# sanderslab/magellanmapper

Measured on AMD Instinct MI355X. Metric: Mvoxels/s, 2048x2048x1024 uint16 stack, 5-sigma LoG blob detection, higher is better.
Workload: dtype f16x2 MFMA (f32 accumulate) + 16-bit fixed-point intermediates; f64 re-score of every candidate

## Files before the change

magellanmapper_amd/csrc/mmx_fused4.hip:

```cpp

#include <algorithm>
#include <type_traits>

#include "mmx_common.h"

typedef _Float16 h2_4 __attribute__((ext_vector_type(2)));
typedef _Float16 h8_4 __attribute__((ext_vector_type(8)));
typedef float f2_4 __attribute__((ext_vector_type(2)));
typedef float f4_4 __attribute__((ext_vector_type(4)));
typedef unsigned u4_4 __attribute__((ext_vector_type(4)));
typedef unsigned u2_4 __attribute__((ext_vector_type(2)));

#define MMX_ZX4_MAXCLS 8
#ifndef ZX4_ST_AUX
#define ZX4_ST_AUX 0
#endif
#ifndef ZX4_LD_AUX
#define ZX4_LD_AUX 0
#endif

struct mmx_zx4_cfg {
    float w0[MMX_MAX_RADIUS_FAST + 1];
    float w2[MMX_MAX_RADIUS_FAST + 1];
    float xscale;
    int radius;
    int ncw, ncz;
    int wcls[MMX_ZX4_MAXCLS];
    int zcls[MMX_ZX4_MAXCLS];
    int maxcol, maxu;
    float qp, qq;
    int staged;
    int ntw;
};

namespace {

#ifndef ZX4_PF
#define ZX4_PF 3
#endif
constexpr int kPF4 = ZX4_PF;
#ifndef ZX6_PF
#define ZX6_PF 2
#endif
constexpr float kLoScale = 2048.f;
constexpr float kLoInv = 1.f / 2048.f;

using rsrc4_t = __amdgpu_buffer_rsrc_t;
__device__ __forceinline__ rsrc4_t make_rsrc4(const void* p)
{
    return __builtin_amdgcn_make_buffer_rsrc(const_cast<void*>(p), 0, 0x7fffffff, 0x00020000);
}

template <int NKX, int LA> struct cls4 {
    static constexpr int R8 = NKX == 1 ? 8 : (LA == 1 ? 16 : 24);
    static __host__ __device__ constexpr int xstart(int c)
    {
        const int lo = 16 * c - R8;
        const int al = lo & ~31;
        return (al + 32 * NKX >= 16 * c + 16 + R8) ? al : lo;
    }
    static constexpr int NKZ = LA + 1;
    static constexpr int NT = 2 * NKZ;
};

__device__ __forceinline__ unsigned pack_h2(float a, float b)
{
    const f2_4 v = {a, b};
    return __builtin_bit_cast(unsigned, __builtin_convertvector(v, h2_4));
}

__device__ __forceinline__ float folded_tap(const float* w, int R, int p, int o, int n)
{
    float s = 0.f;
    int d = p - o; d = d < 0 ? -d : d;
    if (d <= R) s += w[d];
    d = (-1 - p) - o; d = d < 0 ? -d : d;
    if (d <= R) s += w[d];
    d = (2 * n - 1 - p) - o; d = d < 0 ? -d : d;
    if (d <= R) s += w[d];
    return s;
}

template <int NKX, int LA>
__global__ void __launch_bounds__(256)
zx4_setup(mmx_zx4_cfg cfg, u4_4* __restrict__ xtab, u4_4* __restrict__ ztab)
{
    using cg = cls4<NKX, LA>;
    const int R = cfg.radius;
    const int lane = threadIdx.x & 63;
    const int kq = lane >> 4, col = lane & 15;
    const int e = blockIdx.x * 4 + (threadIdx.x >> 6);
    const int nx_entries = cfg.ncw * cfg.maxcol * NKX * 2;
    const int nz_entries = cfg.ncz * cfg.maxu * cg::NKZ * 2;
    float wt[8];
    u4_4* dst;
    if (e < nx_entries) {
        const int kern = e & 1;
        const int m = (e >> 1) % NKX;
        const int c = ((e >> 1) / NKX) % cfg.maxcol;
        const int cl = ((e >> 1) / NKX) / cfg.maxcol;
        const int W = cfg.wcls[cl];
        const float* w = kern ? cfg.w2 : cfg.w0;
        const int xo = 16 * c + col;
        const int cwin = cfg.ntw == 2 ? (c & ~1) : c;
        const int xc = (cfg.staged == 2 ? 16 * cwin - cg::R8 : cg::xstart(c)) + 32 * m + 8 * kq;
        int xl = xc < 0 ? 0 : xc;
        xl = xl > W - 8 ? W - 8 : xl;
        if (cfg.staged) xl = xc;
#pragma unroll
        for (int j = 0; j < 8; ++j) {
            const int p = xl + j;
            const bool ok = p >= xc && p < xc + 8 && p >= 0 && p < W && xo < W;
            wt[j] = ok ? folded_tap(w, R, p, xo, W) * cfg.xscale * (cfg.qp > 0.f ? (kern ? cfg.qq : cfg.qp) : 1.f) : 0.f;
        }
        dst = xtab + (size_t)e * 2 * 64;
    } else if (e < nx_entries + nz_entries) {
        const int ez = e - nx_entries;
        const int kern = ez & 1;
        const int ks = (ez >> 1) % cg::NKZ;
        const int U = ((ez >> 1) / cg::NKZ) % cfg.maxu;
        const int cl = ((ez >> 1) / cg::NKZ) / cfg.maxu;
        const int nz = cfg.zcls[cl];
        const float* w = kern ? cfg.w2 : cfg.w0;
        const int zo = 16 * U + col;
#pragma unroll
        for (int j = 0; j < 8; ++j) {
            const int i = 2 * ks + (j >> 2);
            const int zi = 16 * (U - LA + i) + 4 * kq + (j & 3);
            const bool ok = i < cg::NT - 1 && zi >= 0 && zi < nz && zo < nz;
            wt[j] = ok ? folded_tap(w, R, zi, zo, nz) * (cfg.qp > 0.f && kern ? cfg.qq / cfg.qp : 1.f) : 0.f;
        }
        dst = ztab + (size_t)ez * 2 * 64;
    } else {
        return;
    }
    unsigned hi[4], lo[4];
#pragma unroll
    for (int j = 0; j < 8; j += 2) {
        const f2_4 v = {wt[j], wt[j + 1]};
        const h2_4 h = __builtin_convertvector(v, h2_4);
        const f2_4 r = {(wt[j] - (float)h.x) * kLoScale, (wt[j + 1] - (float)h.y) * kLoScale};
        hi[j >> 1] = __builtin_bit_cast(unsigned, h);
        lo[j >> 1] = __builtin_bit_cast(unsigned, __builtin_convertvector(r, h2_4));
    }
    dst[lane] = (u4_4){hi[0], hi[1], hi[2], hi[3]};
    dst[64 + lane] = (u4_4){lo[0], lo[1], lo[2], lo[3]};
}

template <typename InT> struct pieces4;
template <> struct pieces4<uint16_t> {
    using raw_t = u4_4;
    static __device__ __forceinline__ raw_t load(rsrc4_t r, unsigned off, unsigned soff = 0)
    {
        return __builtin_bit_cast(u4_4, __builtin_amdgcn_raw_buffer_load_b128(r, off, soff, ZX4_LD_AUX));
    }
    static __device__ __forceinline__ void split(const raw_t& d, u4_4& hi, u4_4& lo)
    {
        const h2_4 four = {(_Float16)4.0f, (_Float16)4.0f};
        const h2_4 sixty4th = {(_Float16)0.015625f, (_Float16)0.015625f};
#pragma unroll
        for (int i = 0; i < 4; ++i) {
            const unsigned th = __builtin_amdgcn_perm(0x44004400u, d[i], 0x07030501u);
            const unsigned tl = __builtin_amdgcn_perm(0x24002400u, d[i], 0x07020500u);
            hi[i] = __builtin_bit_cast(unsigned, __builtin_bit_cast(h2_4, th) - four);
            lo[i] = __builtin_bit_cast(unsigned, __builtin_bit_cast(h2_4, tl) - sixty4th);
        }
    }
    static constexpr float kBiasHi = 4.0f, kBiasLo = 0.015625f;
    static __device__ __forceinline__ void split_biased(const raw_t& d, u4_4& hi, u4_4& lo)
    {
#pragma unroll
        for (int i = 0; i < 4; ++i) {
            hi[i] = __builtin_amdgcn_perm(0x44004400u, d[i], 0x07030501u);
            lo[i] = __builtin_amdgcn_perm(0x24002400u, d[i], 0x07020500u);
        }
    }
};

struct presplit_t { u4_4 h, l; };
template <> struct pieces4<float> {
    using raw_t = presplit_t;
    static __device__ __forceinline__ raw_t load(rsrc4_t r, unsigned off, unsigned soff = 0)
    {
        raw_t v;
        v.h = __builtin_bit_cast(u4_4, __builtin_amdgcn_raw_buffer_load_b128(r, off, soff, ZX4_LD_AUX));
        v.l = __builtin_bit_cast(u4_4, __builtin_amdgcn_raw_buffer_load_b128(r, off + 256u, soff, ZX4_LD_AUX));
        return v;
    }
    static __device__ __forceinline__ void split(const raw_t& d, u4_4& hi, u4_4& lo) { hi = d.h; lo = d.l; }
    [[maybe_unused]] static constexpr float kBiasHi = 0.f, kBiasLo = 0.f;
    static __device__ __forceinline__ void split_biased(const raw_t& d, u4_4& hi, u4_4& lo) { hi = d.h; lo = d.l; }
};
template <typename InT> struct is_f32_4 { static constexpr bool value = false; };
template <> struct is_f32_4<float> { static constexpr bool value = true; };
template <typename InT> struct lo_scaled4 { static constexpr bool value = false; };
template <> struct lo_scaled4<float> { static constexpr bool value = true; };

__device__ __forceinline__ f4_4 mfma16(const u4_4& a, const u4_4& b, const f4_4& c)
{
    return __builtin_amdgcn_mfma_f32_16x16x32_f16(__builtin_bit_cast(h8_4, a), __builtin_bit_cast(h8_4, b), c, 0, 0, 0);
}

template <int NKX, int LA, typename InT, bool Q16 = false, int NTW = 1>
__global__ void __launch_bounds__(256, (NTW == 1 && (LA == 1 || Q16) && !is_f32_4<InT>::value) ? 3 : 2)
zx4_kernel(const InT* __restrict__ vol, int64_t stride_z, int64_t stride_y,
           const mmx_block* __restrict__ blocks, int64_t slot_elems,
           float* __restrict__ gp, float* __restrict__ gq,
           const u4_4* __restrict__ xtab, const u4_4* __restrict__ ztab, mmx_zx4_cfg cfg)
{
    using cg = cls4<NKX, LA>;
    using pc = pieces4<InT>;
    constexpr int NKZ = cg::NKZ, NT = cg::NT;
    constexpr int kUnit = std::is_same<InT, float>::value ? 512 : 256;
    constexpr bool LO_SCALED = lo_scaled4<InT>::value;
    static_assert(NTW == 1 || (NTW == 2 && Q16 && NKX == 2 && LA == 1), "two tiles per wave: 16-bit tiles, 8 < radius <= 16");
    constexpr bool ZLDS = LA == 1 || Q16;
    constexpr int PF = ZLDS ? ZX6_PF : kPF4;
    const mmx_block bd = blocks[blockIdx.y];
    const int W = bd.nx, nz = bd.nz;
    const int ntx = (W + 15) >> 4;
    const int bx = (int)(blockIdx.x & 7) * (int)(gridDim.x >> 3) + (int)(blockIdx.x >> 3);
    const int gw = bx * 4 + __builtin_amdgcn_readfirstlane((int)(threadIdx.x >> 6));
    const int ntp = (ntx + NTW - 1) / NTW;
    const int y = gw / ntp;
    const int c = (gw - y * ntp) * NTW;
    const int lane = threadIdx.x & 63;
    const int li = lane & 15, kq = lane >> 4;
    int cw = 0, cz = 0;
    for (int i = 1; i < cfg.ncw; ++i) cw = cfg.wcls[i] == W ? i : cw;
    for (int i = 1; i < cfg.ncz; ++i) cz = cfg.zcls[i] == nz ? i : cz;
    const int ntz = (nz + 15) >> 4;
    const int R = cfg.radius;
    const int u_lo = (R + 15) >> 4;
    const int u_hi = (nz - 16 - R) >> 4;
    const u4_4* zt = ztab + ((size_t)cz * cfg.maxu * NKZ * 2) * 128 + lane;
    constexpr bool ROT = ZLDS && Q16 && NTW == 1 && !is_f32_4<InT>::value && (NKX == 1 || LA == 2);
    constexpr int ZL1 = NKZ * 4 * 64;
    __shared__ u4_4 zl[ZLDS ? (ROT ? 2 : 1) * ZL1 : 1];
    if constexpr (ZLDS) {
        const u4_4* zi = ztab + ((size_t)(cz * cfg.maxu + (u_lo < cfg.maxu ? u_lo : 0)) * NKZ * 2) * 128;
        for (int e = threadIdx.x; e < ZL1; e += 256) zl[e] = zi[e];
        __syncthreads();
        if constexpr (ROT) {
            for (int e = threadIdx.x; e < ZL1; e += 256) {
                const u4_4 cur = zl[e];
                const u4_4 prev = e >= 256 ? zl[e - 256] : (u4_4){0u, 0u, 0u, 0u};
                zl[ZL1 + e] = (u4_4){prev.z, prev.w, cur.x, cur.y};
            }
            __syncthreads();
        }
    }
    if (y >= bd.ny) return;

    u4_4 xw[NTW][NKX][2][2];
    const bool has2 = NTW == 2 && c + 1 < ntx;
#pragma unroll
    for (int i = 0; i < NTW; ++i) {
        const u4_4* xt = xtab + ((size_t)(cw * cfg.maxcol + (i && !has2 ? c : c + i)) * NKX * 2) * 128 + lane;
#pragma unroll
        for (int m = 0; m < NKX; ++m)
#pragma unroll
            for (int k = 0; k < 2; ++k) {
                xw[i][m][k][0] = xt[(m * 2 + k) * 128];
                xw[i][m][k][1] = xt[(m * 2 + k) * 128 + 64];
            }
    }
    constexpr bool BIASED = Q16 && !is_f32_4<InT>::value && LA == 1;
    constexpr bool MIXSPLIT = Q16;
    const f4_4 zero4 = {0.f, 0.f, 0.f, 0.f};
    f4_4 a_start[NTW], b_start[NTW];
#pragma unroll
    for (int i = 0; i < NTW; ++i) { a_start[i] = zero4; b_start[i] = zero4; }
    if constexpr (BIASED) {
        const u4_4 ones = {0x3C003C00u, 0x3C003C00u, 0x3C003C00u, 0x3C003C00u};
#pragma unroll
        for (int i = 0; i < NTW; ++i) {
            f4_4 sh[2] = {zero4, zero4}, sl[2] = {zero4, zero4};
#pragma unroll
            for (int m = 0; m < NKX; ++m)
#pragma unroll
                for (int k = 0; k < 2; ++k) {
                    sh[k] = mfma16(ones, xw[i][m][k][0], sh[k]);
                    sl[k] = mfma16(ones, xw[i][m][k][1], sl[k]);
                }
            const float ca = -((pc::kBiasHi + pc::kBiasLo) * sh[0][0] + pc::kBiasHi * sl[0][0] * kLoInv);
            const float cb = -((pc::kBiasHi + pc::kBiasLo) * sh[1][0] + pc::kBiasHi * sl[1][0] * kLoInv);
            a_start[i] = (f4_4){ca, ca, ca, ca};
            b_start[i] = (f4_4){cb, cb, cb, cb};
        }
    }
    u4_4 zw[ZLDS ? 1 : NKZ][2][2];
    int zset = -1;

    const InT* in = vol + (int64_t)bd.slot * stride_z;
    const int nch8 = (W + 7) >> 3;
    unsigned xoff[NKX];
#pragma unroll
    for (int m = 0; m < NKX; ++m) {
        int j = 2 * c - cg::R8 / 8 + 4 * m + kq;
        j = j < 0 ? 0 : (j > nch8 - 1 ? nch8 - 1 : j);
        xoff[m] = (unsigned)(j * kUnit + li * 16);
    }
    const rsrc4_t rin = make_rsrc4(in);
    auto load_tile = [&](int t, typename pc::raw_t (&raw)[NKX]) __attribute__((always_inline)) {
        const unsigned so = (unsigned)((y * ntz + t) * nch8) * (unsigned)kUnit;
#pragma unroll
        for (int m = 0; m < NKX; ++m) raw[m] = pc::load(rin, xoff[m], so);
    };

    unsigned win[NTW][4][NT][2];
#pragma unroll
    for (int w = 0; w < NTW; ++w)
#pragma unroll
        for (int a = 0; a < 4; ++a)
#pragma unroll
            for (int i = 0; i < NT; ++i) { win[w][a][i][0] = 0u; win[w][a][i][1] = 0u; }

    const unsigned col_b = (unsigned)ntz * 1024u;
    const unsigned live_b = col_b - (unsigned)(16 * ntz - nz) * 64u;
    const int64_t wave_e = (int64_t)((y * ntx + c) * ntz) * 256;
    const rsrc4_t rp = __builtin_amdgcn_make_buffer_rsrc(gp + (int64_t)bd.slot * slot_elems + wave_e, 0, (int)live_b, 0x00020000);
    const rsrc4_t rq = __builtin_amdgcn_make_buffer_rsrc(gq + (int64_t)bd.slot * slot_elems + wave_e, 0, (int)live_b, 0x00020000);
    const rsrc4_t rp2 = __builtin_amdgcn_make_buffer_rsrc(gp + (int64_t)bd.slot * slot_elems + wave_e + (int64_t)ntz * 256, 0,
                                                          has2 ? (int)live_b : 0, 0x00020000);
    const unsigned plane_b = 64u;
    unsigned obase = (unsigned)((4 * li + kq) * 16);

    typename pc::raw_t raw[PF][NKX];
#pragma unroll
    for (int u = 0; u < PF; ++u) load_tile(u < ntz ? u : ntz - 1, raw[u]);

    f4_4 outP[PF][NTW], outQ[PF];
#pragma unroll
    for (int u = 0; u < PF; ++u) {
#pragma unroll
        for (int w = 0; w < NTW; ++w) outP[u][w] = zero4;
        outQ[u] = zero4;
    }
    auto step = [&](int t, auto steady_tag, auto phase_tag, typename pc::raw_t (&rw)[NKX], f4_4 (&P)[NTW], f4_4& Q) __attribute__((always_inline)) {
        constexpr bool STEADY = decltype(steady_tag)::value;
        constexpr int PH = decltype(phase_tag)::value;
        constexpr bool TURN = STEADY && ROT && PH >= 0;
        constexpr int SLOT = TURN ? PH : 2 * LA;
        if constexpr (!TURN) {
#pragma unroll
            for (int w = 0; w < NTW; ++w)
#pragma unroll
                for (int a = 0; a < 4; ++a)
#pragma unroll
                    for (int i = 0; i < 2 * LA; ++i) { win[w][a][i][0] = win[w][a][i + 1][0]; win[w][a][i][1] = win[w][a][i + 1][1]; }
        }
        if (STEADY || t < ntz) {
            u4_4 dh[NKX], dl[NKX];
#pragma unroll
            for (int m = 0; m < NKX; ++m) {
                if constexpr (BIASED) pc::split_biased(rw[m], dh[m], dl[m]);
                else pc::split(rw[m], dh[m], dl[m]);
            }
            __builtin_amdgcn_sched_barrier(0);
            if (STEADY) load_tile(t + PF < ntz ? t + PF : ntz - 1, rw);
            else if (t + PF < ntz) load_tile(t + PF, rw);
            __builtin_amdgcn_sched_barrier(0);
#pragma unroll
            for (int w = 0; w < NTW; ++w) {
                f4_4 a0 = a_start[w], a1 = zero4, b0 = b_start[w], b1 = zero4;
#pragma unroll
                for (int m = 0; m < NKX; ++m) {
                    a0 = mfma16(dh[m], xw[w][m][0][0], a0);
                    b0 = mfma16(dh[m], xw[w][m][1][0], b0);
                    a1 = mfma16(dh[m], xw[w][m][0][1], a1);
                    b1 = mfma16(dh[m], xw[w][m][1][1], b1);
                    if constexpr (LO_SCALED) {
                        a1 = mfma16(dl[m], xw[w][m][0][0], a1);
                        b1 = mfma16(dl[m], xw[w][m][1][0], b1);
                    } else {
                        a0 = mfma16(dl[m], xw[w][m][0][0], a0);
                        b0 = mfma16(dl[m], xw[w][m][1][0], b0);
                        if constexpr (!Q16) {
                            a1 = mfma16(dl[m], xw[w][m][0][1], a1);
                            b1 = mfma16(dl[m], xw[w][m][1][1], b1);
                        }
                    }
                }
#pragma unroll
                for (int r = 0; r < 4; r += 2) {
                    const float av0 = __builtin_fmaf(a1[r], kLoInv, a0[r]), av1 = __builtin_fmaf(a1[r + 1], kLoInv, a0[r + 1]);
                    const float bv0 = __builtin_fmaf(b1[r], kLoInv, b0[r]), bv1 = __builtin_fmaf(b1[r + 1], kLoInv, b0[r + 1]);
                    const f2_4 av = {av0, av1}, bv = {bv0, bv1};
                    const h2_4 ah = __builtin_convertvector(av, h2_4), bh = __builtin_convertvector(bv, h2_4);
                    if constexpr (MIXSPLIT) {
                        const f2_4 ar = {av0 - (float)ah.x, av1 - (float)ah.y}, br = {bv0 - (float)bh.x, bv1 - (float)bh.y};
                        win[w][0][SLOT][r >> 1] = __builtin_bit_cast(unsigned, ah);
                        win[w][1][SLOT][r >> 1] = __builtin_bit_cast(unsigned, __builtin_convertvector(ar, h2_4));
                        win[w][2][SLOT][r >> 1] = __builtin_bit_cast(unsigned, bh);
                        win[w][3][SLOT][r >> 1] = __builtin_bit_cast(unsigned, __builtin_convertvector(br, h2_4));
                        continue;
                    }
                    const f2_4 ar = {__builtin_fmaf((float)ah.x, -kLoScale, av0 * kLoScale), __builtin_fmaf((float)ah.y, -kLoScale, av1 * kLoScale)};
                    const f2_4 br = {__builtin_fmaf((float)bh.x, -kLoScale, bv0 * kLoScale), __builtin_fmaf((float)bh.y, -kLoScale, bv1 * kLoScale)};
                    win[w][0][SLOT][r >> 1] = __builtin_bit_cast(unsigned, ah);
                    win[w][1][SLOT][r >> 1] = __builtin_bit_cast(unsigned, __builtin_convertvector(ar, h2_4));
                    win[w][2][SLOT][r >> 1] = __builtin_bit_cast(unsigned, bh);
                    win[w][3][SLOT][r >> 1] = __builtin_bit_cast(unsigned, __builtin_convertvector(br, h2_4));
                }
            }
        } else {
#pragma unroll
            for (int w = 0; w < NTW; ++w)
#pragma unroll
                for (int a = 0; a < 4; ++a) { win[w][a][SLOT][0] = 0u; win[w][a][SLOT][1] = 0u; }
        }
        const int U = t - LA;
        if (STEADY || U >= 0) {
            const int want = (U >= u_lo && U <= u_hi) ? u_lo : U;
            if constexpr (!STEADY && !ZLDS) {
                if (want != zset) {
                    zset = want;
#pragma unroll
                    for (int ks = 0; ks < NKZ; ++ks)
#pragma unroll
                        for (int k = 0; k < 2; ++k) {
                            zw[ks][k][0] = zt[((size_t)(want * NKZ + ks) * 2 + k) * 128];
                            zw[ks][k][1] = zt[((size_t)(want * NKZ + ks) * 2 + k) * 128 + 64];
                        }
                }
            }
            f4_4 p0[NTW], p1[NTW], q0[NTW], q1[NTW];
#pragma unroll
            for (int w = 0; w < NTW; ++w) { p0[w] = zero4; p1[w] = zero4; q0[w] = zero4; q1[w] = zero4; }
#pragma unroll
            for (int ks = 0; ks < NKZ; ++ks) {
                u4_4 z00, z01, z10, z11;
                if constexpr (!ZLDS) {
                    z00 = zw[ks][0][0]; z01 = zw[ks][0][1]; z10 = zw[ks][1][0]; z11 = zw[ks][1][1];
                } else if constexpr (STEADY) {
                    constexpr int TR = TURN ? (PH - (NT - 2) + NT) % NT : 0;
                    const int KF = ((TR & 1) ? ZL1 : 0) + ((ks - TR / 2 + NKZ) % NKZ) * 256;
                    z00 = zl[KF + 0 * 64 + lane]; z01 = zl[KF + 1 * 64 + lane];
                    z10 = zl[KF + 2 * 64 + lane]; z11 = zl[KF + 3 * 64 + lane];
                } else {
                    const u4_4* zp = zt + ((size_t)(want * NKZ + ks) * 2) * 128;
                    z00 = zp[0]; z01 = zp[64]; z10 = zp[128]; z11 = zp[192];
                }
#pragma unroll
                for (int w = 0; w < NTW; ++w) {
                    const u4_4 ah = {win[w][0][2 * ks][0], win[w][0][2 * ks][1], win[w][0][2 * ks + 1][0], win[w][0][2 * ks + 1][1]};
                    const u4_4 al = {win[w][1][2 * ks][0], win[w][1][2 * ks][1], win[w][1][2 * ks + 1][0], win[w][1][2 * ks + 1][1]};
                    const u4_4 bh = {win[w][2][2 * ks][0], win[w][2][2 * ks][1], win[w][2][2 * ks + 1][0], win[w][2][2 * ks + 1][1]};
                    const u4_4 bl = {win[w][3][2 * ks][0], win[w][3][2 * ks][1], win[w][3][2 * ks + 1][0], win[w][3][2 * ks + 1][1]};
                    p0[w] = mfma16(ah, z00, p0[w]);
                    q0[w] = mfma16(bh, z00, q0[w]);
                    p1[w] = mfma16(ah, z01, p1[w]);
                    q1[w] = mfma16(bh, z01, q1[w]);
                    if constexpr (MIXSPLIT) {
                        p0[w] = mfma16(al, z00, p0[w]);
                        q0[w] = mfma16(bl, z00, q0[w]);
                    } else {
                        p1[w] = mfma16(al, z00, p1[w]);
                        q1[w] = mfma16(bl, z00, q1[w]);
                    }
                    q0[w] = mfma16(ah, z10, q0[w]);
                    q1[w] = mfma16(ah, z11, q1[w]);
                    if constexpr (MIXSPLIT) q0[w] = mfma16(al, z10, q0[w]);
                    else q1[w] = mfma16(al, z10, q1[w]);
                }
                if constexpr (ZLDS && !STEADY) __builtin_amdgcn_sched_barrier(0);
            }
            __builtin_amdgcn_sched_barrier(0);
#pragma unroll
            for (int w = 0; w < NTW; ++w) asm volatile("" ::"v"(P[w]));
            asm volatile("" ::"v"(Q));
            {
                if constexpr (Q16) {
#pragma unroll
                    for (int w = 0; w < NTW; ++w) {
#pragma unroll
                        for (int r = 0; r < 4; r += 2) {
                            const float pa = __builtin_fmaf(p1[w][r], kLoInv, p0[w][r]), pb = __builtin_fmaf(p1[w][r + 1], kLoInv, p0[w][r + 1]);
                            const float qa = __builtin_fmaf(q1[w][r], kLoInv, q0[w][r]), qb = __builtin_fmaf(q1[w][r + 1], kLoInv, q0[w][r + 1]);
                            const unsigned pu = __builtin_bit_cast(unsigned, __builtin_amdgcn_cvt_pknorm_u16(pa, pb));
                            const unsigned qs = __builtin_bit_cast(unsigned, __builtin_amdgcn_cvt_pknorm_i16(qa, qb));
                            const unsigned da = __builtin_amdgcn_perm(qs, pu, 0x05040100u);
                            const unsigned db = __builtin_amdgcn_perm(qs, pu, 0x07060302u);
                            float ra, rb;
                            asm volatile("v_mov_b32 %0, %1" : "=v"(ra) : "v"(__uint_as_float(da)));
                            asm volatile("v_mov_b32 %0, %1" : "=v"(rb) : "v"(__uint_as_float(db)));
                            P[w][r] = ra;
                            P[w][r + 1] = rb;
                        }
                        if (w == 0) __builtin_amdgcn_raw_buffer_store_b128(__builtin_bit_cast(u4_4, P[w]), rp, obase, 0, ZX4_ST_AUX);
                        else __builtin_amdgcn_raw_buffer_store_b128(__builtin_bit_cast(u4_4, P[w]), rp2, obase, 0, ZX4_ST_AUX);
                    }
                } else {
#pragma unroll
                for (int r = 0; r < 4; ++r) {
                    const float pv = __builtin_fmaf(p1[0][r], kLoInv, p0[0][r]);
                    const float qv = __builtin_fmaf(q1[0][r], kLoInv, q0[0][r]);
                    float pr, qr;
                    asm volatile("v_mov_b32 %0, %1" : "=v"(pr) : "v"(pv));
                    asm volatile("v_mov_b32 %0, %1" : "=v"(qr) : "v"(qv));
                    P[0][r] = pr;
                    Q[r] = qr;
                }
                __builtin_amdgcn_raw_buffer_store_b128(__builtin_bit_cast(u4_4, P[0]), rp, obase, 0, ZX4_ST_AUX);
                __builtin_amdgcn_raw_buffer_store_b128(__builtin_bit_cast(u4_4, Q), rq, obase, 0, ZX4_ST_AUX);
                }
            }
            obase += 16u * plane_b;
        }
        __builtin_amdgcn_sched_barrier(0);
    };
    const int t_end = ntz + LA;
    int tA = ((u_lo + LA + PF - 1) / PF) * PF;
    int nB = (u_hi + LA + 1 < ntz ? u_hi + LA + 1 : ntz) - tA;
    constexpr int GROUP = ROT ? NT : PF;
    static_assert(GROUP % PF == 0, "a turn of the window is a whole number of rings");
    nB = nB > 0 ? (nB / GROUP) * GROUP : 0;
    if (tA > t_end) tA = ((t_end + PF - 1) / PF) * PF;
    const int tB = tA + nB;
#pragma unroll 1
    for (int t0 = 0; t0 < tA; t0 += PF) {
#pragma unroll
        for (int u = 0; u < PF; ++u)
            if (t0 + u < t_end) step(t0 + u, std::false_type{}, std::integral_constant<int, -1>{}, raw[u], outP[u], outQ[u]);
    }
    if (nB > 0) {
        if (!ZLDS && zset != u_lo) {
            zset = u_lo;
#pragma unroll
            for (int ks = 0; ks < NKZ; ++ks)
#pragma unroll
                for (int k = 0; k < 2; ++k) {
                    zw[ks][k][0] = zt[((size_t)(u_lo * NKZ + ks) * 2 + k) * 128];
                    zw[ks][k][1] = zt[((size_t)(u_lo * NKZ + ks) * 2 + k) * 128 + 64];
                }
        }
        __builtin_amdgcn_s_waitcnt(0x0F70);
        auto turn = [&](int t0, auto... J) __attribute__((always_inline)) {
            (step(t0 + decltype(J)::value, std::true_type{},
                  std::integral_constant<int, ROT ? (NT - 1 + decltype(J)::value) % NT : -1>{},
                  raw[decltype(J)::value % PF], outP[decltype(J)::value % PF], outQ[decltype(J)::value % PF]), ...);
        };
        if constexpr (!ROT) {
#pragma unroll 1
            for (int t0 = tA; t0 < tB; t0 += PF) {
#pragma unroll
                for (int u = 0; u < PF; ++u) step(t0 + u, std::true_type{}, std::integral_constant<int, -1>{}, raw[u], outP[u], outQ[u]);
            }
        } else {
#pragma unroll 1
            for (int t0 = tA; t0 < tB; t0 += GROUP) {
                using std::integral_constant;
                if constexpr (GROUP == 4) turn(t0, integral_constant<int, 0>{}, integral_constant<int, 1>{}, integral_constant<int, 2>{},
                                               integral_constant<int, 3>{});
                else turn(t0, integral_constant<int, 0>{}, integral_constant<int, 1>{}, integral_constant<int, 2>{},
                          integral_constant<int, 3>{}, integral_constant<int, 4>{}, integral_constant<int, 5>{});
                static_assert(GROUP == 4 || GROUP == 6, "turn lengths built: 4 (radius <= 16), 6 (radius <= 24)");
            }
        }
    }
#pragma unroll 1
    for (int t0 = tB; t0 < t_end; t0 += PF) {
#pragma unroll
        for (int u = 0; u < PF; ++u)
            if (t0 + u < t_end) step(t0 + u, std::false_type{}, std::integral_constant<int, -1>{}, raw[u], outP[u], outQ[u]);
    }
}



template <typename InT>
__global__ void __launch_bounds__(256)
zx6_pack_kernel(const InT* __restrict__ vol, int64_t stride_z, int64_t stride_y, int64_t stride_x,
                const mmx_block* __restrict__ blocks, uint16_t* __restrict__ pack, int64_t pack_stride)
{
    constexpr int PITCH = 512 + 8;
    __shared__ __attribute__((aligned(16))) uint16_t tile[16][PITCH];
    const mmx_block bd = blocks[blockIdx.y];
    const int ntz = (bd.nz + 15) >> 4, nch8 = (bd.nx + 7) >> 3;
    const int yt = blockIdx.x;
    if (yt >= bd.ny * ntz) return;
    const int y = yt / ntz, t = yt - y * ntz;
    const int wave = threadIdx.x >> 6, lane = threadIdx.x & 63;
    const InT* src = vol + bd.src_off + (int64_t)y * stride_y;
    bool quads = false;
    if constexpr (sizeof(InT) == 2)
        quads = stride_x == 1 && ((bd.src_off | stride_y | stride_z) & 3) == 0 && (reinterpret_cast<uintptr_t>(vol) & 7) == 0;
    if (quads) {
        u2_4 v[4][2];
        bool have[4][2];
#pragma unroll
        for (int i = 0; i < 4; ++i) {
            const int z = 16 * t + 4 * wave + i;
            const InT* row = src + (int64_t)(z < bd.nz ? z : 0) * stride_z;
#pragma unroll
            for (int h = 0; h < 2; ++h) {
                const int x = lane * 4 + 256 * h;
                have[i][h] = x < 8 * nch8;
                v[i][h] = (u2_4){0u, 0u};
                if (have[i][h] && z < bd.nz) {
                    if (x + 3 < bd.nx) {
                        v[i][h] = *reinterpret_cast<const u2_4*>(row + x);
                    } else {
                        unsigned e[4];
#pragma unroll
                        for (int j = 0; j < 4; ++j) e[j] = x + j < bd.nx ? (unsigned)row[x + j] : 0u;
                        v[i][h] = (u2_4){e[0] | (e[1] << 16), e[2] | (e[3] << 16)};
                    }
                }
            }
        }
#pragma unroll
        for (int i = 0; i < 4; ++i)
#pragma unroll
            for (int h = 0; h < 2; ++h)
                if (have[i][h]) *reinterpret_cast<u2_4*>(&tile[4 * wave + i][lane * 4 + 256 * h]) = v[i][h];
    } else
#pragma unroll
    for (int i = 0; i < 4; ++i) {
        const int r = 4 * wave + i, z = 16 * t + r;
        if (z >= bd.nz) {
            for (int x = lane * 4; x < 8 * nch8; x += 256) *reinterpret_cast<u2_4*>(&tile[r][x]) = (u2_4){0u, 0u};
        } else {
            for (int x = lane; x < 8 * nch8; x += 64)
                tile[r][x] = x < bd.nx ? (uint16_t)((unsigned)src[(int64_t)z * stride_z + (int64_t)x * stride_x] << (sizeof(InT) == 1 ? 8 : 0))
                                       : (uint16_t)0;
        }
    }
    __syncthreads();
    u4_4* dst = reinterpret_cast<u4_4*>(pack + (int64_t)bd.slot * pack_stride) + (int64_t)yt * nch8 * 16;
    for (int u = threadIdx.x; u < nch8 * 16; u += 256) {
        const int j = u >> 4, r = u & 15;
        dst[u] = *reinterpret_cast<const u4_4*>(&tile[r][8 * j]);
    }
}

__global__ void __launch_bounds__(256)
zx6_pack_f32_kernel(const float* __restrict__ vol, int64_t stride_z, int64_t stride_y, int64_t stride_x,
                    const mmx_block* __restrict__ blocks, uint16_t* __restrict__ pack, int64_t pack_stride)
{
    constexpr int PITCH = 512 + 4;
    __shared__ __attribute__((aligned(16))) unsigned tile[16][PITCH];
    const mmx_block bd = blocks[blockIdx.y];
    const int ntz = (bd.nz + 15) >> 4, nch8 = (bd.nx + 7) >> 3;
    const int yt = blockIdx.x;
    if (yt >= bd.ny * ntz) return;
    const int y = yt / ntz, t = yt - y * ntz;
    const int wave = threadIdx.x >> 6, lane = threadIdx.x & 63;
    const float* src = vol + bd.src_off + (int64_t)y * stride_y;
    auto pieces = [](float v) __attribute__((always_inline)) {
        const _Float16 h = (_Float16)v;
        const _Float16 l = (_Float16)((v - (float)h) * kLoScale);
        return (unsigned)__builtin_bit_cast(unsigned short, h) | ((unsigned)__builtin_bit_cast(unsigned short, l) << 16);
    };
    const bool quads = stride_x == 1 && ((bd.src_off | stride_y | stride_z) & 3) == 0 && (reinterpret_cast<uintptr_t>(vol) & 15) == 0;
#pragma unroll
    for (int i = 0; i < 4; ++i) {
        const int r = 4 * wave + i, z = 16 * t + r;
        if (quads && z < bd.nz) {
            const float* row = src + (int64_t)z * stride_z;
            for (int x = lane * 4; x < 8 * nch8; x += 256) {
                f4_4 v = {0.f, 0.f, 0.f, 0.f};
                if (x + 3 < bd.nx) v = *reinterpret_cast<const f4_4*>(row + x);
                else
                    for (int j = 0; j < 4; ++j) v[j] = x + j < bd.nx ? row[x + j] : 0.f;
                *reinterpret_cast<u4_4*>(&tile[r][x]) = (u4_4){pieces(v[0]), pieces(v[1]), pieces(v[2]), pieces(v[3])};
            }
        } else {
            for (int x = lane; x < 8 * nch8; x += 64) {
                float v = 0.f;
                if (z < bd.nz && x < bd.nx) v = src[(int64_t)z * stride_z + (int64_t)x * stride_x];
                tile[r][x] = pieces(v);
            }
        }
    }
    __syncthreads();
    u4_4* dst = reinterpret_cast<u4_4*>(pack + (int64_t)bd.slot * pack_stride) + (int64_t)yt * nch8 * 32;
    for (int u = threadIdx.x; u < nch8 * 16; u += 256) {
        const int j = u >> 4, r = u & 15;
        const u4_4 a = *reinterpret_cast<const u4_4*>(&tile[r][8 * j]);
        const u4_4 b = *reinterpret_cast<const u4_4*>(&tile[r][8 * j + 4]);
        const u4_4 hi = {__builtin_amdgcn_perm(a[1], a[0], 0x05040100u), __builtin_amdgcn_perm(a[3], a[2], 0x05040100u),
                         __builtin_amdgcn_perm(b[1], b[0], 0x05040100u), __builtin_amdgcn_perm(b[3], b[2], 0x05040100u)};
        const u4_4 lo = {__builtin_amdgcn_perm(a[1], a[0], 0x07060302u), __builtin_amdgcn_perm(a[3], a[2], 0x07060302u),
                         __builtin_amdgcn_perm(b[1], b[0], 0x07060302u), __builtin_amdgcn_perm(b[3], b[2], 0x07060302u)};
        dst[j * 32 + r] = hi;
        dst[j * 32 + 16 + r] = lo;
    }
}

struct zx_classes {
    int ncw, ncz, wcls[MMX_ZX4_MAXCLS], zcls[MMX_ZX4_MAXCLS];
    int maxcol, maxu;
};
bool collect_classes(const mmx_block* h_blocks, int n_blocks, zx_classes* c)
{
    c->ncw = c->ncz = c->maxcol = c->maxu = 0;
    for (int i = 0; i < n_blocks; ++i) {
        const mmx_block& b = h_blocks[i];
        int j;
        for (j = 0; j < c->ncw && c->wcls[j] != b.nx; ++j) {}
        if (j == c->ncw) { if (j == MMX_ZX4_MAXCLS) return false; c->wcls[c->ncw++] = b.nx; }
        for (j = 0; j < c->ncz && c->zcls[j] != b.nz; ++j) {}
        if (j == c->ncz) { if (j == MMX_ZX4_MAXCLS) return false; c->zcls[c->ncz++] = b.nz; }
        c->maxcol = std::max(c->maxcol, (b.nx + 15) / 16);
        c->maxu = std::max(c->maxu, (b.nz + 15) / 16);
    }
    return true;
}

template <int NKX, int LA>
int launch_zx6(const mmx_volume* vol, const mmx_block* d_blocks, const mmx_block* h_blocks, int n_blocks,
               const mmx_zx6_plan& plan, const mmx_taps_f32& tx, int radius, void* d_work, float qp, float qq, hipStream_t s)
{
    using cg = cls4<NKX, LA>;
    mmx_zx4_cfg cfg{};
    for (int k = 0; k <= MMX_MAX_RADIUS_FAST; ++k) { cfg.w0[k] = tx.w0[k]; cfg.w2[k] = tx.w2[k]; }
    cfg.radius = radius;
    cfg.xscale = vol->dtype == MMX_U16 ? (float)(65536.0 / 65535.0) :
                 (vol->dtype == MMX_U8 ? (float)(65536.0 / (255.0 * 256.0)) : 1.f);
    cfg.staged = 2;
    cfg.qp = qp; cfg.qq = qq;
    const bool pair = NKX == 2 && LA == 1 && qp > 0.f && vol->dtype != MMX_F32;
    cfg.ntw = pair ? 2 : 1;
    zx_classes cl;
    if (!collect_classes(h_blocks, n_blocks, &cl)) return MMX_ERR_UNSUPPORTED;
    cfg.ncw = cl.ncw; cfg.ncz = cl.ncz; cfg.maxcol = cl.maxcol; cfg.maxu = cl.maxu;
    for (int j = 0; j < MMX_ZX4_MAXCLS; ++j) {
        cfg.wcls[j] = j < cl.ncw ? cl.wcls[j] : -1;
        cfg.zcls[j] = j < cl.ncz ? cl.zcls[j] : -1;
    }
    int max_waves = 0;
    for (int i = 0; i < n_blocks; ++i) {
        const mmx_block& b = h_blocks[i];
        if (b.nx < radius || b.nz < radius) return MMX_ERR_UNSUPPORTED;
        const int ntx = (b.nx + 15) / 16;
        max_waves = std::max(max_waves, b.ny * (pair ? (ntx + 1) / 2 : ntx));
    }
    const int nx_entries = cfg.ncw * cfg.maxcol * NKX * 2;
    const int nz_entries = cfg.ncz * cfg.maxu * cg::NKZ * 2;
    const size_t xbytes = (size_t)nx_entries * 2 * 64 * sizeof(u4_4);
    const size_t zbytes = (size_t)nz_entries * 2 * 64 * sizeof(u4_4);
    if ((int64_t)(xbytes + zbytes) > plan.tab_bytes) return MMX_ERR_UNSUPPORTED;
    char* w = reinterpret_cast<char*>(d_work);
    u4_4* xtab = reinterpret_cast<u4_4*>(w + plan.tab_off);
    u4_4* ztab = reinterpret_cast<u4_4*>(w + plan.tab_off + xbytes);
    hipLaunchKernelGGL((zx4_setup<NKX, LA>), dim3((nx_entries + nz_entries + 3) / 4), dim3(256), 0, s, cfg, xtab, ztab);
    dim3 grid((((max_waves + 3) / 4) + 7) & ~7, n_blocks);
    if (vol->dtype == MMX_F32) {
        if (qp > 0.f)
            hipLaunchKernelGGL((zx4_kernel<NKX, LA, float, true>), grid, dim3(256), 0, s,
                               reinterpret_cast<const float*>(w + plan.pack_off), plan.pack_stride / 2, (int64_t)0, d_blocks,
                               plan.tile_stride, reinterpret_cast<float*>(w), reinterpret_cast<float*>(w + plan.q_off),
                               xtab, ztab, cfg);
        else
            hipLaunchKernelGGL((zx4_kernel<NKX, LA, float, false>), grid, dim3(256), 0, s,
                               reinterpret_cast<const float*>(w + plan.pack_off), plan.pack_stride / 2, (int64_t)0, d_blocks,
                               plan.tile_stride, reinterpret_cast<float*>(w), reinterpret_cast<float*>(w + plan.q_off),
                               xtab, ztab, cfg);
    } else if (pair) {
        if constexpr (NKX == 2 && LA == 1)
            hipLaunchKernelGGL((zx4_kernel<NKX, LA, uint16_t, true, 2>), grid, dim3(256), 0, s,
                               reinterpret_cast<const uint16_t*>(w + plan.pack_off), plan.pack_stride, (int64_t)0, d_blocks,
                               plan.tile_stride, reinterpret_cast<float*>(w), reinterpret_cast<float*>(w + plan.q_off),
                               xtab, ztab, cfg);
    } else if (qp > 0.f)
        hipLaunchKernelGGL((zx4_kernel<NKX, LA, uint16_t, true>), grid, dim3(256), 0, s,
                           reinterpret_cast<const uint16_t*>(w + plan.pack_off), plan.pack_stride, (int64_t)0, d_blocks,
                           plan.tile_stride, reinterpret_cast<float*>(w), reinterpret_cast<float*>(w + plan.q_off),
                           xtab, ztab, cfg);
    else
        hipLaunchKernelGGL((zx4_kernel<NKX, LA, uint16_t, false>), grid, dim3(256), 0, s,
                           reinterpret_cast<const uint16_t*>(w + plan.pack_off), plan.pack_stride, (int64_t)0, d_blocks,
                           plan.tile_stride, reinterpret_cast<float*>(w), reinterpret_cast<float*>(w + plan.q_off),
                           xtab, ztab, cfg);
    return hipGetLastError() == hipSuccess ? MMX_OK : MMX_ERR_HIP;
}

}

int mmx_zx6_plan_make(const mmx_block* h_blocks, int n_blocks, int64_t slot_elems, int voxel_dtype, mmx_zx6_plan* plan)
{
    const int pieces = voxel_dtype == MMX_F32 ? 2 : 1;
    int64_t tile = 0, pk = 0;
    int max_tiles = 0, max_rowtiles = 0;
    zx_classes cl;
    if (!collect_classes(h_blocks, n_blocks, &cl)) return MMX_ERR_UNSUPPORTED;
    for (int i = 0; i < n_blocks; ++i) {
        const mmx_block& b = h_blocks[i];
        if (b.px > 512) return MMX_ERR_UNSUPPORTED;
        const int ntx = (b.nx + 15) / 16, ntz = (b.nz + 15) / 16, nch8 = (b.nx + 7) / 8;
        const int64_t te = (int64_t)ntx * ntz * b.ny * 256, pe = (int64_t)b.ny * ntz * nch8 * 128 * pieces;
        if (te > tile) tile = te;
        if (pe > pk) pk = pe;
        if (ntx * ntz > max_tiles) max_tiles = ntx * ntz;
        if (b.ny * ntz > max_rowtiles) max_rowtiles = b.ny * ntz;
    }
    if (tile * 4 >= (int64_t(1) << 31) || pk * 2 >= (int64_t(1) << 31)) return MMX_ERR_UNSUPPORTED;
    plan->tile_stride = tile;
    plan->pack_stride = pk;
    plan->q_off = (int64_t)n_blocks * tile * 4;
    plan->tab_off = 2 * plan->q_off;
    plan->tab_bytes = (int64_t)(cl.ncw * cl.maxcol * 2 * 2 + cl.ncz * cl.maxu * 3 * 2) * 2 * 64 * 16;
    plan->pack_off = (plan->tab_off + plan->tab_bytes + 255) & ~int64_t(255);
    plan->max_tiles = max_tiles;
    plan->max_rowtiles = max_rowtiles;
    const int64_t need = plan->pack_off + (int64_t)n_blocks * pk * 2;
    return need <= 4 * (int64_t)n_blocks * slot_elems * 4 ? MMX_OK : MMX_ERR_UNSUPPORTED;
}

int mmx_launch_zx6_pack(const mmx_volume* vol, const mmx_block* d_blocks, const mmx_block* h_blocks, int n_blocks,
                        const mmx_zx6_plan& plan, void* d_work, hipStream_t stream)
{
    (void)h_blocks;
    if (vol->dtype != MMX_U16 && vol->dtype != MMX_U8 && vol->dtype != MMX_F32) return MMX_ERR_UNSUPPORTED;
    uint16_t* pack = reinterpret_cast<uint16_t*>(reinterpret_cast<char*>(d_work) + plan.pack_off);
    dim3 grid(plan.max_rowtiles, n_blocks);
    if (vol->dtype == MMX_F32)
        hipLaunchKernelGGL(zx6_pack_f32_kernel, grid, dim3(256), 0, stream, (const float*)vol->d_data,
                           vol->stride_z, vol->stride_y, vol->stride_x, d_blocks, pack, plan.pack_stride);
    else if (vol->dtype == MMX_U16)
        hipLaunchKernelGGL((zx6_pack_kernel<uint16_t>), grid, dim3(256), 0, stream, (const uint16_t*)vol->d_data,
                           vol->stride_z, vol->stride_y, vol->stride_x, d_blocks, pack, plan.pack_stride);
    else
        hipLaunchKernelGGL((zx6_pack_kernel<uint8_t>), grid, dim3(256), 0, stream, (const uint8_t*)vol->d_data,
                           vol->stride_z, vol->stride_y, vol->stride_x, d_blocks, pack, plan.pack_stride);
    return hipGetLastError() == hipSuccess ? MMX_OK : MMX_ERR_HIP;
}

int mmx_launch_zx6(const mmx_volume* vol, const mmx_block* d_blocks, const mmx_block* h_blocks, int n_blocks,
                   const mmx_zx6_plan& plan, const mmx_taps_f32& tx, int radius, void* d_work, float qp, float qq,
                   hipStream_t stream)
{
    if (vol->dtype != MMX_U16 && vol->dtype != MMX_U8 && vol->dtype != MMX_F32) return MMX_ERR_UNSUPPORTED;
    if (radius < 1 || radius > MMX_MAX_RADIUS_FAST) return MMX_ERR_UNSUPPORTED;
    if (radius <= 8) return launch_zx6<1, 1>(vol, d_blocks, h_blocks, n_blocks, plan, tx, radius, d_work, qp, qq, stream);
    if (radius <= 16) return launch_zx6<2, 1>(vol, d_blocks, h_blocks, n_blocks, plan, tx, radius, d_work, qp, qq, stream);
    return launch_zx6<2, 2>(vol, d_blocks, h_blocks, n_blocks, plan, tx, radius, d_work, qp, qq, stream);
}
```

Measured before the change: 43900.

## Stage edge z-tap tables in dynamic LDS and use buffer loads otherwise

Moves the z-weight table to dynamically sized shared memory and, alongside the inner set, preloads the boundary (edge) z tap sets each block needs. Non-steady edge tiles then read from LDS instead of global memory, with a buffer-load fallback plus waitcnt when the sets do not fit the LDS cap. The launch path now sizes LDS per variant through a helper, which can raise LDS use and lower occupancy, and adds a per-block prologue copy.

```diff
diff --git a/magellanmapper_amd/csrc/mmx_fused4.hip b/magellanmapper_amd/csrc/mmx_fused4.hip
--- a/magellanmapper_amd/csrc/mmx_fused4.hip
+++ b/magellanmapper_amd/csrc/mmx_fused4.hip
@@ -31,6 +31,7 @@
     float qp, qq;
     int staged;
     int ntw;
+    int zsets;
 };
 
 namespace {
@@ -236,10 +237,20 @@
     const u4_4* zt = ztab + ((size_t)cz * cfg.maxu * NKZ * 2) * 128 + lane;
     constexpr bool ROT = ZLDS && Q16 && NTW == 1 && !is_f32_4<InT>::value && (NKX == 1 || LA == 2);
     constexpr int ZL1 = NKZ * 4 * 64;
-    __shared__ u4_4 zl[ZLDS ? (ROT ? 2 : 1) * ZL1 : 1];
+    constexpr int ZBASE = ROT ? 2 : 1;
+    extern __shared__ u4_4 zl[];
+    const int z_ntop = u_hi >= u_lo ? ntz - 1 - u_hi : 0;
+    const int z_nedge = u_hi >= u_lo ? u_lo + z_ntop : ntz;
+    const int z_nres = ZLDS ? (z_nedge < cfg.zsets - ZBASE ? z_nedge : cfg.zsets - ZBASE) : 0;
     if constexpr (ZLDS) {
-        const u4_4* zi = ztab + ((size_t)(cz * cfg.maxu + (u_lo < cfg.maxu ? u_lo : 0)) * NKZ * 2) * 128;
+        const u4_4* zc = ztab + ((size_t)cz * cfg.maxu * NKZ * 2) * 128;
+        const u4_4* zi = zc + (size_t)(u_lo < cfg.maxu ? u_lo : 0) * ZL1;
         for (int e = threadIdx.x; e < ZL1; e += 256) zl[e] = zi[e];
+        for (int e = threadIdx.x; e < z_nres * ZL1; e += 256) {
+            const int si = e / ZL1, r = e - si * ZL1;
+            const int U = si < z_ntop ? u_hi + 1 + si : si - z_ntop;
+            zl[(ZBASE + si) * ZL1 + r] = zc[(size_t)U * ZL1 + r];
+        }
         __syncthreads();
         if constexpr (ROT) {
             for (int e = threadIdx.x; e < ZL1; e += 256) {
@@ -337,6 +348,11 @@
         for (int w = 0; w < NTW; ++w) outP[u][w] = zero4;
         outQ[u] = zero4;
     }
+    const rsrc4_t rz = make_rsrc4(ztab + ((size_t)cz * cfg.maxu * NKZ * 2) * 128);
+    const unsigned zlane = (unsigned)lane * 16u;
+    auto zfrag = [&](unsigned soff) __attribute__((always_inline)) {
+        return __builtin_bit_cast(u4_4, __builtin_amdgcn_raw_buffer_load_b128(rz, zlane, soff, 0));
+    };
     auto step = [&](int t, auto steady_tag, auto phase_tag, typename pc::raw_t (&rw)[NKX], f4_4 (&P)[NTW], f4_4& Q) __attribute__((always_inline)) {
         constexpr bool STEADY = decltype(steady_tag)::value;
         constexpr int PH = decltype(phase_tag)::value;
@@ -428,20 +444,7 @@
             f4_4 p0[NTW], p1[NTW], q0[NTW], q1[NTW];
 #pragma unroll
             for (int w = 0; w < NTW; ++w) { p0[w] = zero4; p1[w] = zero4; q0[w] = zero4; q1[w] = zero4; }
-#pragma unroll
-            for (int ks = 0; ks < NKZ; ++ks) {
-                u4_4 z00, z01, z10, z11;
-                if constexpr (!ZLDS) {
-                    z00 = zw[ks][0][0]; z01 = zw[ks][0][1]; z10 = zw[ks][1][0]; z11 = zw[ks][1][1];
-                } else if constexpr (STEADY) {
-                    constexpr int TR = TURN ? (PH - (NT - 2) + NT) % NT : 0;
-                    const int KF = ((TR & 1) ? ZL1 : 0) + ((ks - TR / 2 + NKZ) % NKZ) * 256;
-                    z00 = zl[KF + 0 * 64 + lane]; z01 = zl[KF + 1 * 64 + lane];
-                    z10 = zl[KF + 2 * 64 + lane]; z11 = zl[KF + 3 * 64 + lane];
-                } else {
-                    const u4_4* zp = zt + ((size_t)(want * NKZ + ks) * 2) * 128;
-                    z00 = zp[0]; z01 = zp[64]; z10 = zp[128]; z11 = zp[192];
-                }
+            auto zmac = [&](int ks, const u4_4& z00, const u4_4& z01, const u4_4& z10, const u4_4& z11) __attribute__((always_inline)) {
 #pragma unroll
                 for (int w = 0; w < NTW; ++w) {
                     const u4_4 ah = {win[w][0][2 * ks][0], win[w][0][2 * ks][1], win[w][0][2 * ks + 1][0], win[w][0][2 * ks + 1][1]};
@@ -464,7 +467,35 @@
                     if constexpr (MIXSPLIT) q0[w] = mfma16(al, z10, q0[w]);
                     else q1[w] = mfma16(al, z10, q1[w]);
                 }
-                if constexpr (ZLDS && !STEADY) __builtin_amdgcn_sched_barrier(0);
+            };
+            if constexpr (!ZLDS) {
+#pragma unroll
+                for (int ks = 0; ks < NKZ; ++ks) zmac(ks, zw[ks][0][0], zw[ks][0][1], zw[ks][1][0], zw[ks][1][1]);
+            } else if constexpr (STEADY) {
+#pragma unroll
+                for (int ks = 0; ks < NKZ; ++ks) {
+                    constexpr int TR = TURN ? (PH - (NT - 2) + NT) % NT : 0;
+                    const int KF = ((TR & 1) ? ZL1 : 0) + ((ks - TR / 2 + NKZ) % NKZ) * 256;
+                    zmac(ks, zl[KF + 0 * 64 + lane], zl[KF + 1 * 64 + lane], zl[KF + 2 * 64 + lane], zl[KF + 3 * 64 + lane]);
+                }
+            } else {
+                const bool inner = U >= u_lo && U <= u_hi;
+                const int ei = (u_hi >= u_lo && U > u_hi) ? U - u_hi - 1 : z_ntop + U;
+                const bool zres = inner || ei < z_nres;
+                const u4_4* zp = zl + __builtin_amdgcn_readfirstlane(inner ? 0 : (ZBASE + ei) * ZL1) + lane;
+#pragma unroll
+                for (int ks = 0; ks < NKZ; ++ks) {
+                    u4_4 z00, z01, z10, z11;
+                    if (zres) {
+                        z00 = zp[ks * 256]; z01 = zp[ks * 256 + 64]; z10 = zp[ks * 256 + 128]; z11 = zp[ks * 256 + 192];
+                    } else {
+                        const unsigned so = (unsigned)((want * NKZ + ks) * 4096);
+                        z00 = zfrag(so); z01 = zfrag(so + 1024u); z10 = zfrag(so + 2048u); z11 = zfrag(so + 3072u);
+                        __builtin_amdgcn_s_waitcnt(0x0F70);
+                    }
+                    zmac(ks, z00, z01, z10, z11);
+                    __builtin_amdgcn_sched_barrier(0);
+                }
             }
             __builtin_amdgcn_sched_barrier(0);
 #pragma unroll
@@ -709,6 +740,33 @@
     return true;
 }
 
+template <int NKX, int LA, typename InT, bool Q16, int NTW>
+hipError_t launch_zx4(dim3 grid, hipStream_t s, const zx_classes& cl, mmx_zx4_cfg cfg, const void* pack, int64_t pack_stride,
+                      const mmx_block* d_blocks, int64_t tile_stride, float* gp, float* gq, const u4_4* xtab, const u4_4* ztab)
+{
+    constexpr bool F32 = is_f32_4<InT>::value;
+    constexpr bool ZLDS = LA == 1 || Q16;
+    constexpr bool ROT = ZLDS && Q16 && NTW == 1 && !F32 && (NKX == 1 || LA == 2);
+    constexpr int WGS = LA == 1 ? (NTW == 2 ? 2 : 4) : (Q16 && !F32 ? 3 : 2);
+    constexpr size_t kSet = (size_t)(LA + 1) * 4096;
+    constexpr size_t kCap = std::min<size_t>(160 * 1024 / WGS, 64 * 1024) / kSet * kSet;
+    size_t lds = 0;
+    if (ZLDS) {
+        const int base = ROT ? 2 : 1, u_lo = (cfg.radius + 15) >> 4;
+        cfg.zsets = base;
+        for (int j = 0; j < cl.ncz; ++j) {
+            const int nz = cl.zcls[j], ntz = (nz + 15) >> 4, u_hi = (nz - 16 - cfg.radius) >> 4;
+            cfg.zsets = std::max(cfg.zsets, base + (u_hi >= u_lo ? u_lo + (ntz - 1 - u_hi) : ntz));
+        }
+        cfg.zsets = std::min(cfg.zsets, (int)(kCap / kSet));
+        lds = cfg.zsets * kSet;
+    }
+    auto kern = zx4_kernel<NKX, LA, InT, Q16, NTW>;
+    hipLaunchKernelGGL(kern, grid, dim3(256), lds, s, reinterpret_cast<const InT*>(pack), pack_stride, (int64_t)0, d_blocks,
+                       tile_stride, gp, gq, xtab, ztab, cfg);
+    return hipGetLastError();
+}
+
 template <int NKX, int LA>
 int launch_zx6(const mmx_volume* vol, const mmx_block* d_blocks, const mmx_block* h_blocks, int n_blocks,
                const mmx_zx6_plan& plan, const mmx_taps_f32& tx, int radius, void* d_work, float qp, float qq, hipStream_t s)
@@ -747,33 +805,23 @@
     u4_4* ztab = reinterpret_cast<u4_4*>(w + plan.tab_off + xbytes);
     hipLaunchKernelGGL((zx4_setup<NKX, LA>), dim3((nx_entries + nz_entries + 3) / 4), dim3(256), 0, s, cfg, xtab, ztab);
     dim3 grid((((max_waves + 3) / 4) + 7) & ~7, n_blocks);
+    const void* pk = w + plan.pack_off;
+    float* gp = reinterpret_cast<float*>(w);
+    float* gq = reinterpret_cast<float*>(w + plan.q_off);
+    hipError_t e;
     if (vol->dtype == MMX_F32) {
-        if (qp > 0.f)
-            hipLaunchKernelGGL((zx4_kernel<NKX, LA, float, true>), grid, dim3(256), 0, s,
-                               reinterpret_cast<const float*>(w + plan.pack_off), plan.pack_stride / 2, (int64_t)0, d_blocks,
-                               plan.tile_stride, reinterpret_cast<float*>(w), reinterpret_cast<float*>(w + plan.q_off),
-                               xtab, ztab, cfg);
-        else
-            hipLaunchKernelGGL((zx4_kernel<NKX, LA, float, false>), grid, dim3(256), 0, s,
-                               reinterpret_cast<const float*>(w + plan.pack_off), plan.pack_stride / 2, (int64_t)0, d_blocks,
-                               plan.tile_stride, reinterpret_cast<float*>(w), reinterpret_cast<float*>(w + plan.q_off),
-                               xtab, ztab, cfg);
+        if (qp > 0.f) e = launch_zx4<NKX, LA, float, true, 1>(grid, s, cl, cfg, pk, plan.pack_stride / 2, d_blocks, plan.tile_stride, gp, gq, xtab, ztab);
+        else e = launch_zx4<NKX, LA, float, false, 1>(grid, s, cl, cfg, pk, plan.pack_stride / 2, d_blocks, plan.tile_stride, gp, gq, xtab, ztab);
     } else if (pair) {
         if constexpr (NKX == 2 && LA == 1)
-            hipLaunchKernelGGL((zx4_kernel<NKX, LA, uint16_t, true, 2>), grid, dim3(256), 0, s,
-                               reinterpret_cast<const uint16_t*>(w + plan.pack_off), plan.pack_stride, (int64_t)0, d_blocks,
-                               plan.tile_stride, reinterpret_cast<float*>(w), reinterpret_cast<float*>(w + plan.q_off),
-                               xtab, ztab, cfg);
+            e = launch_zx4<NKX, LA, uint16_t, true, 2>(grid, s, cl, cfg, pk, plan.pack_stride, d_blocks, plan.tile_stride, gp, gq, xtab, ztab);
+        else
+            e = hipErrorInvalidValue;
     } else if (qp > 0.f)
-        hipLaunchKernelGGL((zx4_kernel<NKX, LA, uint16_t, true>), grid, dim3(256), 0, s,
-                           reinterpret_cast<const uint16_t*>(w + plan.pack_off), plan.pack_stride, (int64_t)0, d_blocks,
-                           plan.tile_stride, reinterpret_cast<float*>(w), reinterpret_cast<float*>(w + plan.q_off),
-                           xtab, ztab, cfg);
+        e = launch_zx4<NKX, LA, uint16_t, true, 1>(grid, s, cl, cfg, pk, plan.pack_stride, d_blocks, plan.tile_stride, gp, gq, xtab, ztab);
     else
-        hipLaunchKernelGGL((zx4_kernel<NKX, LA, uint16_t, false>), grid, dim3(256), 0, s,
-                           reinterpret_cast<const uint16_t*>(w + plan.pack_off), plan.pack_stride, (int64_t)0, d_blocks,
-                           plan.tile_stride, reinterpret_cast<float*>(w), reinterpret_cast<float*>(w + plan.q_off),
-                           xtab, ztab, cfg);
+        e = launch_zx4<NKX, LA, uint16_t, false, 1>(grid, s, cl, cfg, pk, plan.pack_stride, d_blocks, plan.tile_stride, gp, gq, xtab, ztab);
+    if (e != hipSuccess) return MMX_ERR_HIP;
     return hipGetLastError() == hipSuccess ? MMX_OK : MMX_ERR_HIP;
 }
 
```

Measured after the change: 44220 (median of 6 runs). About the same (+0.7%).
